# gopi-erabati/Object-Pose-Estimation

Measured on NVIDIA B200. Metric: frames_per_sec_fpfh_sacia_icp_640x480, higher is better.
Workload: dtype f32

## Files before the change

object-pose-estimation_b200/csrc/registration.cu:

```cuda
#include <cooperative_groups.h>

#include <algorithm>
#include <cmath>
#include <cstdlib>

#include <map>
#include <mutex>

#include <chrono>
#include "ope_host.cuh"
#include "ope_octet.cuh"

namespace cg = cooperative_groups;

namespace ope {

__global__ void transform_kernel(const float4* __restrict__ in, const float4* __restrict__ in_n, int n, Mat4 T,
                                 float4* __restrict__ out, float4* __restrict__ out_n) {
  int i = blockIdx.x * blockDim.x + threadIdx.x;
  if (i >= n) return;
  float4 p = __ldg(in + i);
  float4 o = p;
  xform_point(T, p.x, p.y, p.z, o.x, o.y, o.z);
  out[i] = o;
// ... 201 lines not shown
  float cert_gap;
  int dfs_max;
  int tgt_in_smem;
  int n_tgt;
  int split_min;
  int small_max;
  float4* def_q;
  int4* def_m;
  float4* def_res;
  int* def_count;
  int* def_head;
  double* partials;
  unsigned* barrier;
  ope_reg_result* result;
  long long* phase_cycles;
  Mat4 guess;
};

static constexpr int kIcpThreads = 512;
static constexpr int kIcpWarps = kIcpThreads / 32;
static constexpr int kIcpAcc = 17;
static constexpr int kIcpMaxBlocks = 1024;
static constexpr int kIcpSmemMaxTargets = 4096;
static constexpr int kIcpSplitMin = 6144;


struct IcpSmem {
  OctStack wstack[kIcpWarps];
  float2 knn_buf[kIcpWarps][kKnnBufCap + 32];
  LeafList leaves[kIcpWarps];
  int dir[kDirEntries];
  Nn1Smem<kIcpThreads> nn;
  double red[kIcpWarps][kIcpAcc];
  double totals[kIcpAcc];
  int prefix[2][kIcpMaxBlocks];
  int warp_cnt[2][kIcpWarps];
  int n_def[2];
  Mat4 T_inc;
  int stop;
};

__device__ __forceinline__ void grid_barrier(unsigned* counter, unsigned target) {
  __syncthreads();
  if (threadIdx.x == 0) {
    asm volatile("red.release.gpu.global.add.u32 [%0], 1;" ::"l"(counter) : "memory");
    unsigned v;
    do {
      asm volatile("ld.acquire.gpu.global.u32 %0, [%1];" : "=r"(v) : "l"(counter) : "memory");
    } while (v < target);
  }
  __syncthreads();
}

__device__ __forceinline__ double warp_reduce16(const double* v, int lane, int& slot) {
  double w8[8], w4[4], w2[2], w1;
  const bool b16 = lane & 16, b8 = lane & 8, b4 = lane & 4, b2 = lane & 2;
#pragma unroll
  for (int j = 0; j < 8; ++j) {
    const double keep = b16 ? v[j + 8] : v[j], give = b16 ? v[j] : v[j + 8];
    w8[j] = keep + __shfl_xor_sync(0xffffffffu, give, 16);
  }
#pragma unroll
  for (int j = 0; j < 4; ++j) {
    const double keep = b8 ? w8[j + 4] : w8[j], give = b8 ? w8[j] : w8[j + 4];
    w4[j] = keep + __shfl_xor_sync(0xffffffffu, give, 8);
  }
#pragma unroll
  for (int j = 0; j < 2; ++j) {
    const double keep = b4 ? w4[j + 2] : w4[j], give = b4 ? w4[j] : w4[j + 2];
    w2[j] = keep + __shfl_xor_sync(0xffffffffu, give, 4);
  }
  {
    const double keep = b2 ? w2[1] : w2[0], give = b2 ? w2[0] : w2[1];
    w1 = keep + __shfl_xor_sync(0xffffffffu, give, 2);
  }
  w1 += __shfl_xor_sync(0xffffffffu, w1, 1);
  slot = (b16 ? 8 : 0) + (b8 ? 4 : 0) + (b4 ? 2 : 0) + (b2 ? 1 : 0);
  return w1;
}

__device__ __forceinline__ double moment_term(int e, const float4 p, const float4 t, float d2, const double o[3]) {
  if (e == 0) return 1.0;
  if (e < 4) return e == 1 ? (double)p.x - o[0] : (e == 2 ? (double)p.y - o[1] : (double)p.z - o[2]);
  if (e < 7) return e == 4 ? (double)t.x - o[0] : (e == 5 ? (double)t.y - o[1] : (double)t.z - o[2]);
  if (e < 16) {
    const int c = (e - 7) / 3, r = (e - 7) % 3;
    const double sv = c == 0 ? (double)p.x - o[0] : (c == 1 ? (double)p.y - o[1] : (double)p.z - o[2]);
    const double tv = r == 0 ? (double)t.x - o[0] : (r == 1 ? (double)t.y - o[1] : (double)t.z - o[2]);
    return tv * sv;
  }
  return (double)d2;
}

__device__ __forceinline__ int icp_reject(const IcpDev& a, int s, int orig, const float4 p, int match) {
  const bool stale = a.variant == OPE_ICP_VARIANT_MODCORR;
  for (int r = 0; r < a.n_rej && match >= 0; ++r) {
    const float4 sn = stale ? __ldg(a.src0_nrm + orig) : a.cur_nrm[s];
    double score;
    if (a.rej_kind[r] == OPE_REJ_SURFACE_NORMAL) {
      const float4 tn = __ldg(a.tgt_nrm + match);
      score = (double)((sn.x * tn.x) + (sn.y * tn.y) + (sn.z * tn.z));
    } else {
      const float4 sp = stale ? __ldg(a.src0_pts + orig) : p;
      const double sl = (double)sqrtf(sp.x * sp.x + sp.y * sp.y + sp.z * sp.z);
      score = (double)((sn.x * (-sp.x / sl)) + (sn.y * (-sp.y / sl)) + (sn.z * (-sp.z / sl)));
    }
    if (!(score > a.rej_thr[r])) match = -1;
  }
  return match;
}

__device__ __forceinline__ int icp_gate(const IcpDev& a, int s, int orig, const float4 p, int nn, float d2) {
  int match = nn;
  if (match >= 0 && (double)d2 > a.max_corr_dist * a.max_corr_dist) match = -1;
  if (match >= 0) match = icp_reject(a, s, orig, p, match);
  return match;
}

__device__ __forceinline__ int icp_correspond_shooting(const IcpDev& a, OctStack* st, int s, int orig, const float4 p, bool use_seed,
                                                       float& d2_out, const float4* tg_smem = nullptr, float2* knn_buf = nullptr) {
  const unsigned full = 0xffffffffu;
  const int lane = threadIdx.x & 31;
  const bool ok = finite3(p.x, p.y, p.z);
  const bool stale = a.variant == OPE_ICP_VARIANT_MODCORR;
  const int k = a.k_search < a.grid.n ? a.k_search : a.grid.n;
  float bound = FLT_MAX;
  if (use_seed && ok) {
    int pj = -1;
    if (lane < k) pj = a.seed[(size_t)s * a.k_search + lane];
    float d = 0.0f;
    if (pj >= 0) { const float4 t = tg_smem ? tg_smem[pj] : __ldg(a.tgt_pts + pj); d = dist2(p.x, p.y, p.z, t.x, t.y, t.z); }
// ... 410 lines not shown
            const double cos_angle = 0.5 * (double)(T(0, 0) + T(1, 1) + T(2, 2) - 1);
            const double translation_sqr = (double)(T(0, 3) * T(0, 3) + T(1, 3) * T(1, 3) + T(2, 3) * T(2, 3));
            int hit = 0, hit_state = 0;
            if (cos_angle >= a.rot_thr && translation_sqr <= a.trans_thr) { hit = 1; hit_state = OPE_CONV_TRANSFORM; }
            else {
              cur_mse = sm->totals[16] / (double)n_corr;
              if (fabs(cur_mse - prev_mse) < a.abs_mse_thr) { hit = 1; hit_state = OPE_CONV_ABS_MSE; }
              else if (fabs(cur_mse - prev_mse) / prev_mse < a.rel_mse_thr) { hit = 1; hit_state = OPE_CONV_REL_MSE; }
              else prev_mse = cur_mse;
            }
            if (hit) {
              if (similar < a.max_similar) ++similar;
              else { similar = 0; state = hit_state; conv = 1; }
            }
          }
          converged = conv;
          if (a.force_all && iterations < a.max_iterations) conv = 0;
          if (conv) stop = 1;
        }
      }
      if (lane == 0) sm->stop = stop;
    }
    __syncthreads();
    if (prof) { const long long t1 = clock64(); t_phase[5] += t1 - t0; t0 = t1; }
    const int stop = sm->stop;
    if (stop != 2) {
      const Mat4 T = sm->T_inc;
      if (!shooting) { for (int s = lo + (int)threadIdx.x; s < hi; s += kIcpThreads) icp_move(a, T, s); }
      else { for (int s = wlo + lane; s < whi; s += 32) icp_move(a, T, s); __syncwarp(); }
    }
    if (prof) {
      const long long t1 = clock64(); t_phase[6] += t1 - t0;
      if (pass < 64) for (int k = 0; k < 7; ++k) { a.phase_cycles[16 + pass * 8 + k] = t_phase[k] - t_prev[k]; t_prev[k] = t_phase[k]; }
    }
    if (stop) break;
  }
  if (prof) {
    for (int i = 0; i < 7; ++i) a.phase_cycles[i] = t_phase[i];
    a.phase_cycles[7] = n_far;
  }
  if (blockIdx.x == 0 && threadIdx.x == 0) {
    ope_reg_result r;
    for (int i = 0; i < 16; ++i) r.T[i] = final_t.m[i];
    r.converged = converged; r.state = state; r.iterations = iterations; r.n_correspondences = n_corr;
    r.last_mse = cur_mse; r.best_error = 0.0; r.best_iteration = 0; r.reserved = 0;
    *a.result = r;
  }
}

static constexpr int kSlabSlots = 32;
static constexpr int kIcpSmallMaxBlocks = 32;

static constexpr int kIcpSmallThreads = 128;
template <int THREADS>
__device__ __forceinline__ void heap_sift(float2* column, int i, float2 v, const int n) {
  for (;;) {
    const int l = 2 * i + 1;
    if (l >= n) break;
    float2 cv = column[l * THREADS];
    int pick = l;
    if (l + 1 < n) {
      const float2 cr = column[(l + 1) * THREADS];
      if (nb_less(cv.x, __float_as_int(cv.y), cr.x, __float_as_int(cr.y))) { cv = cr; pick = l + 1; }
    }
    if (!nb_less(v.x, __float_as_int(v.y), cv.x, __float_as_int(cv.y))) break;
    column[i * THREADS] = cv;
    i = pick;
  }
  column[i * THREADS] = v;
}

template <int THREADS>
struct IcpSmallSmem {
  double red[THREADS / 32][kIcpAcc];
  double totals[kIcpAcc];
  float2 knn_buf[THREADS / 32][kKnnBufCap + 32];
  float4 wbox[THREADS / 32][2];
  Mat4 T_inc;
  int stop;
};

template <int THREADS>
__device__ __forceinline__ void icp_small_body(const IcpDev& a, const int bid, const int nblk) {
  constexpr int kIcpThreads = THREADS, kIcpWarps = THREADS / 32;
  extern __shared__ __align__(16) unsigned char smem_raw[];
  double morg[3];
  { const float4 t0 = a.n_tgt > 0 ? __ldg(a.tgt_pts) : make_float4(0, 0, 0, 0); moment_origin(t0.x, t0.y, t0.z, morg[0], morg[1], morg[2]); }
  IcpSmallSmem<THREADS>* sm = reinterpret_cast<IcpSmallSmem<THREADS>*>(smem_raw);
  float4* tg = reinterpret_cast<float4*>(smem_raw + ((sizeof(IcpSmallSmem<THREADS>) + 15) & ~(size_t)15));
  const int n_tgt8 = (a.n_tgt + 7) & ~7, n_groups = n_tgt8 >> 3;
  float4* blo = tg + n_tgt8;
  float4* bhi = blo + n_groups;
  float2* slab = reinterpret_cast<float2*>(bhi + n_groups);
  const unsigned full = 0xffffffffu;
  const int tid = threadIdx.x, lane = tid & 31, warp = tid >> 5;
  const int s = bid * kIcpThreads + tid;
  const bool in_range = s < a.n_work;
  const bool stale = a.variant == OPE_ICP_VARIANT_MODCORR;
  const int k = a.k_search < a.grid.n ? a.k_search : a.grid.n;
  auto col = [&](int slot) -> float2& { return slab[slot * kIcpThreads + tid]; };

  float4 p = make_float4(0, 0, 0, 0), nv = make_float4(0, 0, 0, 0);
  int orig = 0;
  if (in_range) {
    p = __ldg(a.src_sorted + s);
    orig = __float_as_int(p.w);
    if (a.src0_nrm) nv = __ldg(a.src0_nrm + orig);
    if (!mat4_is_identity(a.guess)) {
      float x, y, z;
      xform_point(a.guess, p.x, p.y, p.z, x, y, z);
      p.x = x; p.y = y; p.z = z;
      if (a.src0_nrm && finite3(nv.x, nv.y, nv.z)) { xform_normal(a.guess, nv.x, nv.y, nv.z, x, y, z); nv.x = x; nv.y = y; nv.z = z; }
    }
  }
  for (int j = tid; j < n_tgt8; j += kIcpThreads) tg[j] = j < a.n_tgt ? __ldg(a.tgt_pts + j) : make_float4(INFINITY, INFINITY, INFINITY, 0.0f);
  __syncthreads();
  for (int g = tid; g < n_groups; g += kIcpThreads) {
    float4 lo = make_float4(INFINITY, INFINITY, INFINITY, 0.0f), hi = make_float4(-INFINITY, -INFINITY, -INFINITY, 0.0f);
    for (int u = 0; u < 8; ++u) {
      const float4 t = tg[8 * g + u];
      if (!finite3(t.x, t.y, t.z)) continue;
      lo.x = fminf(lo.x, t.x); lo.y = fminf(lo.y, t.y); lo.z = fminf(lo.z, t.z);
      hi.x = fmaxf(hi.x, t.x); hi.y = fmaxf(hi.y, t.y); hi.z = fmaxf(hi.z, t.z);
    }
    blo[g] = lo; bhi[g] = hi;
  }
  __syncthreads();
  const bool ok = in_range && k > 0 && finite3(p.x, p.y, p.z);

  Mat4 final_t = a.guess;
  double prev_mse = DBL_MAX, cur_mse = DBL_MAX;
  int similar = 0, iterations = 0, state = OPE_CONV_NOT_CONVERGED, converged = 0, n_corr = 0;
  unsigned bar_target = 0;
  const bool prof = a.phase_cycles != nullptr && bid == 0 && tid == 0;
  long long t_phase[4] = {0, 0, 0, 0};

  auto coop_query = [&](int q, float bound) {
    const float qx = __shfl_sync(full, p.x, q), qy = __shfl_sync(full, p.y, q), qz = __shfl_sync(full, p.z, q);
    float ld; int li;
    const int cnt = warp_knn_smem_bounded(tg, a.n_tgt, a.grid.n, true, qx, qy, qz, a.k_search, bound, sm->knn_buf[warp], ld, li);
    float2* c = slab + (warp * 32 + q);
    if (lane < kSlabSlots) c[lane * kIcpThreads] = lane < cnt ? make_float2(ld, __int_as_float(li)) : make_float2(FLT_MAX, __int_as_float(-1));
    return cnt;
  };

  for (int pass = 0;; ++pass) {
    long long t0 = prof ? clock64() : 0;
    int c = 0;
    bool have = false;
    bool seeded = pass > 0;
    if (pass == 0) {
      const bool leader = (lane & 7) == 0;
      const unsigned lead = __ballot_sync(full, ok && leader);
      for (unsigned m = lead; m != 0u; m &= m - 1u) { const int q = __ffs(m) - 1; const int cnt = coop_query(q, FLT_MAX); if (lane == q) { c = cnt; have = true; } }
      __syncwarp();
      seeded = !leader && ((lead >> (lane & ~7)) & 1u);
    }
    float bound = FLT_MAX;
    if (ok && !have && seeded) {
      const float2* seed_col = slab + (pass == 0 ? (tid & ~7) : tid);
      float b = 0.0f;
      bool all = true;
#pragma unroll 4
      for (int j = 0; j < k; ++j) {
        const int idx = __float_as_int(seed_col[j * kIcpThreads].y);
        if (idx < 0) { all = false; continue; }
        const float4 t = tg[idx];
        b = fmaxf(b, dist2(p.x, p.y, p.z, t.x, t.y, t.z));
      }
      if (all) bound = b;
    }
    if (pass == 0) __syncwarp();
    const bool scan = ok && !have && bound < FLT_MAX;
    int n_ins = 0;
    bool heaped = false;
    float2 root = make_float2(0.0f, 0.0f);
    const long long ts0 = a.phase_cycles ? clock64() : 0;
    if (__any_sync(full, scan)) {
      auto insert_full = [&](float d2, int j) {
        ++n_ins;
        if (!heaped) {
          for (int i = kSlabSlots / 2 - 1; i >= 0; --i) heap_sift<THREADS>(slab + tid, i, col(i), kSlabSlots);
          heaped = true;
          root = col(0);
          bound = root.x;
        }
        if (nb_less(d2, j, root.x, __float_as_int(root.y))) {
          heap_sift<THREADS>(slab + tid, 0, make_float2(d2, __int_as_float(j)), kSlabSlots);
          root = col(0);
          bound = root.x;
        }
      };
      float wlx = scan ? p.x : INFINITY, wly = scan ? p.y : INFINITY, wlz = scan ? p.z : INFINITY;
      float whx = scan ? p.x : -INFINITY, why = scan ? p.y : -INFINITY, whz = scan ? p.z : -INFINITY;
      float wb = scan ? bound : 0.0f;
#pragma unroll
      for (int o = 16; o > 0; o >>= 1) {
        wlx = fminf(wlx, __shfl_xor_sync(full, wlx, o)); wly = fminf(wly, __shfl_xor_sync(full, wly, o)); wlz = fminf(wlz, __shfl_xor_sync(full, wlz, o));
        whx = fmaxf(whx, __shfl_xor_sync(full, whx, o)); why = fmaxf(why, __shfl_xor_sync(full, why, o)); whz = fmaxf(whz, __shfl_xor_sync(full, whz, o));
        wb = fmaxf(wb, __shfl_xor_sync(full, wb, o));
      }
      if (lane == 0) { sm->wbox[warp][0] = make_float4(wlx, wly, wlz, wb * 1.0002f + 1e-30f); sm->wbox[warp][1] = make_float4(whx, why, whz, 0.0f); }
      __syncwarp();
      for (int g0 = 0; g0 < n_groups; g0 += 32) {
        bool near = false;
        if (g0 + lane < n_groups) {
          const float4 lo = blo[g0 + lane], hi = bhi[g0 + lane], wl = sm->wbox[warp][0], wh = sm->wbox[warp][1];
          const float ex = fmaxf(fmaxf(lo.x - wh.x, wl.x - hi.x), 0.0f), ey = fmaxf(fmaxf(lo.y - wh.y, wl.y - hi.y), 0.0f),
                      ez = fmaxf(fmaxf(lo.z - wh.z, wl.z - hi.z), 0.0f);
          near = ex * ex + ey * ey + ez * ez <= wl.w;
        }
        for (unsigned cand = __ballot_sync(full, near); cand != 0u; cand &= cand - 1u) {
          const int g = g0 + __ffs(cand) - 1;
          const int j0 = 8 * g;
          bool mine = scan;
          if (mine) {
            const float4 lo = blo[g], hi = bhi[g];
            const float ex = fmaxf(fmaxf(lo.x - p.x, p.x - hi.x), 0.0f), ey = fmaxf(fmaxf(lo.y - p.y, p.y - hi.y), 0.0f),
                        ez = fmaxf(fmaxf(lo.z - p.z, p.z - hi.z), 0.0f);
            mine = ex * ex + ey * ey + ez * ez <= bound * 1.0001f + 1e-30f;
          }
          if (!mine) continue;
          float d2[8];
#pragma unroll
          for (int u = 0; u < 8; ++u) { const float4 t = tg[j0 + u]; d2[u] = dist2(p.x, p.y, p.z, t.x, t.y, t.z); }
          unsigned hit = 0u;
#pragma unroll
          for (int u = 0; u < 8; ++u) hit |= (d2[u] <= bound ? 1u : 0u) << u;
          if (hit == 0u) continue;
          if (c + __popc(hit) <= kSlabSlots) {
#pragma unroll
            for (int u = 0; u < 8; ++u)
              if ((hit >> u) & 1u) { col(c) = make_float2(d2[u], __int_as_float(j0 + u)); ++c; }
          } else {
#pragma unroll
            for (int u = 0; u < 8; ++u) {
              const bool h = (hit >> u) & 1u;
              const bool room = c < kSlabSlots;
              if (h & room) col(c) = make_float2(d2[u], __int_as_float(j0 + u));
              if (h & !room) insert_full(d2[u], j0 + u);
              c += (h & room) ? 1 : 0;
            }
          }
        }
      }
    }
    const bool unserved = ok && !have && (!scan || c < k);
    const unsigned redo = __ballot_sync(full, unserved);
    if (a.phase_cycles && pass < 64) {
      unsigned long long* pc = (unsigned long long*)(a.phase_cycles + 16 + pass * 8);
      const unsigned long long dt = (unsigned long long)(clock64() - ts0);
      if (lane == 0) { atomicAdd(pc + 0, dt); atomicMax(pc + 1, dt); atomicAdd(pc + 5, 1ull); }
      if (n_ins > 0) { atomicAdd(pc + 2, (unsigned long long)n_ins); atomicAdd(pc + 3, 1ull); }
      if (ok) atomicAdd(pc + 4, (unsigned long long)c);
    }
    if (a.phase_cycles && bid == 0 && lane == 0 && pass > 0) atomicAdd((unsigned long long*)&a.phase_cycles[4], (unsigned long long)__popc(redo));
    if (a.phase_cycles && bid == 0 && ok && pass > 0) atomicAdd((unsigned long long*)&a.phase_cycles[5], (unsigned long long)c);
    for (unsigned m = redo; m != 0u; m &= m - 1u) {
      const int q = __ffs(m) - 1;
      const float bq = __shfl_sync(full, scan ? bound : FLT_MAX, q);
      const int cnt = coop_query(q, bq);
      if (lane == q) c = cnt;
    }
    __syncwarp();
    if (prof) { const long long t1 = clock64(); t_phase[0] += t1 - t0; t0 = t1; }
    int match = -1;
    float d2m = 0.0f;
    if (ok && c > 0) {
      const float4 nr = stale ? __ldg(a.src0_nrm + orig) : nv;
      const double N0 = nr.x, N1 = nr.y, N2 = nr.z;
      double best = DBL_MAX;
      int best_idx = -1, first_idx = -1;
      float best_d2 = 0.0f, first_d2 = 0.0f;
      while (heaped && c > k) {
        --c;
        if (c > 0) heap_sift<THREADS>(slab + tid, 0, col(c), c);
      }
      while (c > k) {
        int worst = 0;
        float2 wv = col(0);
        for (int e = 1; e < c; ++e) { const float2 o = col(e); if (nb_less(wv.x, __float_as_int(wv.y), o.x, __float_as_int(o.y))) { wv = o; worst = e; } }
        --c;
        if (worst != c) col(worst) = col(c);
      }
      float best_key = 0.0f;
#pragma unroll 4
      for (int e = 0; e < c; ++e) {
        const float2 mine = col(e);
        const int mi = __float_as_int(mine.y);
        if (first_idx < 0 || nb_less(mine.x, mi, first_d2, first_idx)) { first_idx = mi; first_d2 = mine.x; }
        const float4 t = tg[mi];
        const float px = t.x - p.x, py = t.y - p.y, pz = t.z - p.z;
        const double V0 = px, V1 = py, V2 = pz;
        const double C0 = N1 * V2 - N2 * V1, C1 = N2 * V0 - N0 * V2, C2 = N0 * V1 - N1 * V0;
        const double dist = C0 * C0 + C1 * C1 + C2 * C2;
        if (dist < DBL_MAX && (dist < best || (dist == best && nb_less(mine.x, mi, best_key, best_idx)))) {
          best = dist; best_idx = mi; best_d2 = mine.x; best_key = mine.x;
        }
      }
      const int pick_idx = best_idx < 0 ? first_idx : best_idx;
      const float pick_d2 = best_idx < 0 ? first_d2 : best_d2;
      const double min_dist = best_idx < 0 ? DBL_MAX : best;
      if (!(min_dist > a.max_corr_dist)) { match = pick_idx; d2m = pick_d2; }
      for (int r = 0; r < a.n_rej && match >= 0; ++r) {
        const float4 sn = stale ? __ldg(a.src0_nrm + orig) : nv;
        double score;
        if (a.rej_kind[r] == OPE_REJ_SURFACE_NORMAL) {
          const float4 tn = __ldg(a.tgt_nrm + match);
          score = (double)((sn.x * tn.x) + (sn.y * tn.y) + (sn.z * tn.z));
        } else {
          const float4 sp = stale ? __ldg(a.src0_pts + orig) : p;
          const double sl = (double)sqrtf(sp.x * sp.x + sp.y * sp.y + sp.z * sp.z);
          score = (double)((sn.x * (-sp.x / sl)) + (sn.y * (-sp.y / sl)) + (sn.z * (-sp.z / sl)));
        }
        if (!(score > a.rej_thr[r])) match = -1;
      }
    }
    if (ok) for (int j = (c < k ? c : k); j < k; ++j) col(j) = make_float2(FLT_MAX, __int_as_float(-1));
    if (in_range) { a.corr_match[orig] = match; a.corr_d2[orig] = d2m; }
    if (prof) { const long long t1 = clock64(); t_phase[1] += t1 - t0; t0 = t1; }
    {
      double v[16];
#pragma unroll
      for (int e = 0; e < 16; ++e) v[e] = 0.0;
      double dsum = 0.0;
      if (match >= 0) {
        const float4 t = tg[match];
#pragma unroll
        for (int e = 0; e < 16; ++e) v[e] = moment_term(e, p, t, d2m, morg);
        dsum = (double)d2m;
      }
      int slot;
      const double wsum = warp_reduce16(v, lane, slot);
      dsum = warp_sum_d(dsum);
      if ((lane & 1) == 0) sm->red[warp][slot] = wsum;
      if (lane == 1) sm->red[warp][16] = dsum;
    }
    __syncthreads();
    double* my_partials = a.partials + ((size_t)(pass & 1) * nblk + bid) * kIcpAcc;
    if (tid < kIcpAcc) {
      double sum = 0.0;
#pragma unroll
      for (int wv = 0; wv < kIcpWarps; ++wv) sum += sm->red[wv][tid];
      my_partials[tid] = sum;
    }
    if (nblk > 1) { bar_target += nblk; grid_barrier(a.barrier, bar_target); } else __syncthreads();
    if (tid < kIcpAcc) {
      const double* base = a.partials + (size_t)(pass & 1) * nblk * kIcpAcc;
      double sum = 0.0;
      for (int b0 = 0; b0 < nblk; b0 += 8) {
        double v[8];
#pragma unroll
        for (int u = 0; u < 8; ++u) v[u] = b0 + u < nblk ? __ldcg(base + (size_t)(b0 + u) * kIcpAcc + tid) : 0.0;
#pragma unroll
        for (int u = 0; u < 8; ++u) sum += v[u];
      }
      sm->totals[tid] = sum;
    }
    __syncthreads();
    if (prof) { const long long t1 = clock64(); t_phase[2] += t1 - t0; t0 = t1; }
    if (tid == 0) {
      int stop = 0;
      n_corr = (int)sm->totals[0];
      if (n_corr < a.min_corr) {
        state = OPE_CONV_NO_CORRESPONDENCES; converged = 0; stop = 2;
        sm->T_inc = mat4_identity();
      } else {
        Mat4 T;
        umeyama_from_moments(sm->totals, T, morg[0], morg[1], morg[2]);
        sm->T_inc = T;
        final_t = mat4_mul(T, final_t);
        ++iterations;
        state = OPE_CONV_NOT_CONVERGED;
        int conv = 0;
        if (iterations >= a.max_iterations) {
          if (!a.fail_after_max) { state = OPE_CONV_ITERATIONS; conv = 1; }
          else { conv = 0; stop = 1; }
        } else {
          const double cos_angle = 0.5 * (double)(T(0, 0) + T(1, 1) + T(2, 2) - 1);
          const double translation_sqr = (double)(T(0, 3) * T(0, 3) + T(1, 3) * T(1, 3) + T(2, 3) * T(2, 3));
          int hit = 0, hit_state = 0;
          if (cos_angle >= a.rot_thr && translation_sqr <= a.trans_thr) { hit = 1; hit_state = OPE_CONV_TRANSFORM; }
          else {
            cur_mse = sm->totals[16] / (double)n_corr;
            if (fabs(cur_mse - prev_mse) < a.abs_mse_thr) { hit = 1; hit_state = OPE_CONV_ABS_MSE; }
            else if (fabs(cur_mse - prev_mse) / prev_mse < a.rel_mse_thr) { hit = 1; hit_state = OPE_CONV_REL_MSE; }
            else prev_mse = cur_mse;
          }
          if (hit) {
            if (similar < a.max_similar) ++similar;
            else { similar = 0; state = hit_state; conv = 1; }
          }
        }
        converged = conv;
        if (a.force_all && iterations < a.max_iterations) conv = 0;
        if (conv) stop = 1;
      }
      sm->stop = stop;
    }
    __syncthreads();
    const int stop = sm->stop;
    if (stop != 2 && in_range && finite3(p.x, p.y, p.z)) {
      const Mat4 T = sm->T_inc;
      float x, y, z;
      xform_point(T, p.x, p.y, p.z, x, y, z);
      p.x = x; p.y = y; p.z = z;
      if (a.src0_nrm && finite3(nv.x, nv.y, nv.z)) { xform_normal(T, nv.x, nv.y, nv.z, x, y, z); nv.x = x; nv.y = y; nv.z = z; }
    }
    if (prof) { const long long t1 = clock64(); t_phase[3] += t1 - t0; }
    if (stop) break;
  }
  if (prof) for (int i = 0; i < 4; ++i) a.phase_cycles[i] = t_phase[i];
  if (bid == 0 && tid == 0) {
    ope_reg_result r;
    for (int i = 0; i < 16; ++i) r.T[i] = final_t.m[i];
    r.converged = converged; r.state = state; r.iterations = iterations; r.n_correspondences = n_corr;
    r.last_mse = cur_mse; r.best_error = 0.0; r.best_iteration = 0; r.reserved = 0;
    *a.result = r;
  }
}

template <int THREADS>
__global__ void __launch_bounds__(THREADS, 512 / THREADS) icp_small_kernel(IcpDev a) {
  icp_small_body<THREADS>(a, (int)blockIdx.x, (int)gridDim.x);
}
template <int THREADS>
__global__ void __launch_bounds__(THREADS, 512 / THREADS) icp_small_batch_kernel(const IcpDev* __restrict__ descs, const int2* __restrict__ map,
                                                                                unsigned* ticket) {
  __shared__ int s_ticket;
  __shared__ IcpDev s_desc;
  if (threadIdx.x == 0) s_ticket = (int)atomicAdd(ticket, 1u);
  __syncthreads();
  const int2 fb = map[s_ticket];
  for (int w = threadIdx.x; w < (int)(sizeof(IcpDev) / 4); w += THREADS) reinterpret_cast<int*>(&s_desc)[w] = reinterpret_cast<const int*>(descs + fb.x)[w];
  __syncthreads();
  icp_small_body<THREADS>(s_desc, fb.y, (s_desc.n_work + THREADS - 1) / THREADS);
}

__global__ void __launch_bounds__(kIcpThreads, 1) correspond_once_kernel(IcpDev a) {
  extern __shared__ __align__(16) unsigned char smem_raw[];
  IcpSmem* sm = reinterpret_cast<IcpSmem*>(smem_raw);
  const int lane = threadIdx.x & 31, warp = threadIdx.x >> 5;
  if (a.estimator != OPE_EST_NORMAL_SHOOTING) {
    for (int base = blockIdx.x * kIcpThreads; base < a.n_src; base += gridDim.x * kIcpThreads) {
      const int i = base + (int)threadIdx.x;
      const bool in_range = i < a.n_src;
      float4 p = make_float4(0, 0, 0, 0);
      if (in_range) p = a.cur_pts[i];
      const bool ok = in_range && finite3(p.x, p.y, p.z);
      float d2 = 0.0f;
      const int nn = block_nn1<kIcpThreads>(a.grid, &sm->nn, ok, p.x, p.y, p.z, a.max_d2_f, -1, nullptr, d2);
      if (in_range) {
        const int m = ok ? icp_gate(a, i, i, p, nn, d2) : -1;
        a.corr_match[i] = m; a.corr_d2[i] = d2;
      }
    }
  } else {
    OctStack* st = &sm->wstack[warp];
    for (int i = blockIdx.x * kIcpWarps + warp; i < a.n_src; i += gridDim.x * kIcpWarps) {
      const float4 p = a.cur_pts[i];
      float d2 = 0.0f;
      const int m = icp_correspond_shooting(a, st, i, i, p, false, d2);
      if (lane == 0) { a.corr_match[i] = m; a.corr_d2[i] = d2; }
      __syncwarp();
    }
  }
}

__global__ void __launch_bounds__(kIcpThreads, 1) reciprocal_filter_kernel(GridView gsrc, const float4* __restrict__ tgt_pts, int* match,
                                                                           int n, float max_d2_f, double max_corr_dist) {
  extern __shared__ __align__(16) unsigned char smem_raw[];
  IcpSmem* sm = reinterpret_cast<IcpSmem*>(smem_raw);
  for (int base = blockIdx.x * kIcpThreads; base < n; base += gridDim.x * kIcpThreads) {
    const int i = base + (int)threadIdx.x;
    const int m = i < n ? match[i] : -1;
    float4 q = make_float4(0, 0, 0, 0);
    if (m >= 0) q = __ldg(tgt_pts + m);
    const bool ok = m >= 0 && finite3(q.x, q.y, q.z);
    float d2 = 0.0f;
    const int back = block_nn1<kIcpThreads>(gsrc, &sm->nn, ok, q.x, q.y, q.z, max_d2_f, -1, nullptr, d2);
// ... 544 lines not shown
}

static int icp_stepwise_device(ope_ctx* ctx, const ope_cloud* src, const ope_cloud* tgt, const ope_icp_params& prm, const Mat4& guess,
                               ope_reg_result* res, ope_correspondence* out_corr_host, ope_cloud** out_aligned,
                               ope_correspondence* fixed = nullptr, size_t n_fixed = 0);

int icp_device(ope_ctx* ctx, const ope_cloud* src, const ope_cloud* tgt, const ope_icp_params& prm, const Mat4& guess,
               ope_reg_result* res, ope_correspondence* out_corr_host, ope_cloud** out_aligned) {
  if (prm.transformation != OPE_TE_SVD || prm.use_reciprocal)
    return icp_stepwise_device(ctx, src, tgt, prm, guess, res, out_corr_host, out_aligned);
  IcpDev a;
  std::memset(&a, 0, sizeof(a));
  OPE_TRY(icp_fill(ctx, src, tgt, prm, &a, true));
  a.guess = guess;
  size_t smem_bytes = ((sizeof(IcpSmem) + 15) & ~(size_t)15) + (a.tgt_in_smem ? tgt->n * sizeof(float4) : 0);
  const size_t n = src->n;
  GridView gsrc;
  std::memset(&gsrc, 0, sizeof(gsrc));
  if (n > 0) OPE_TRY(cloud_any_grid(ctx, src, &gsrc));
  a.src_sorted = gsrc.pts;
  a.n_work = gsrc.n;
  const size_t nw = (size_t)a.n_work;
  ope_cloud* work = nullptr;
  OPE_TRY(cloud_alloc(ctx, std::max<size_t>(n, 1), src->normals != nullptr, &work));
  work->n = n;
  a.cur_pts = work->pts; a.cur_nrm = work->normals;
  Scratch<int> match(ctx), seed(ctx), dcount(ctx), dhead(ctx);
  Scratch<float> d2(ctx);
  Scratch<float4> defq(ctx), refs(ctx), defres(ctx);
  Scratch<int4> defm(ctx);
  Scratch<double> partials(ctx);
  Scratch<unsigned> bar(ctx);
  Scratch<ope_reg_result> dres(ctx);
  const bool shooting = prm.estimator == OPE_EST_NORMAL_SHOOTING;
  int rc = match.alloc(n);
  if (rc == OPE_OK) rc = d2.alloc(n);
  if (rc == OPE_OK) rc = seed.alloc(shooting ? nw * (size_t)prm.k_search : nw);
  if (rc == OPE_OK && !shooting) rc = defq.alloc(nw);
  if (rc == OPE_OK && !shooting) rc = defm.alloc(nw);
  if (rc == OPE_OK && !shooting) rc = refs.alloc(nw);
  if (rc == OPE_OK && !shooting) rc = defres.alloc(nw);
  if (rc == OPE_OK) rc = dres.alloc(1);
  if (rc == OPE_OK) rc = bar.alloc(1);
  if (rc == OPE_OK && cudaMemsetAsync(bar.p, 0, sizeof(unsigned), ctx->stream) != cudaSuccess) rc = fail(ctx, OPE_ERR_CUDA, "memset failed");
  if (rc == OPE_OK && n > 0 && cudaMemsetAsync(match.p, 0xff, n * sizeof(int), ctx->stream) != cudaSuccess) rc = fail(ctx, OPE_ERR_CUDA, "memset failed");
  if (rc == OPE_OK && n > 0 && cudaMemsetAsync(d2.p, 0, n * sizeof(float), ctx->stream) != cudaSuccess) rc = fail(ctx, OPE_ERR_CUDA, "memset failed");
  const char* small_env = std::getenv("OPE_ICP_SMALL");
  const bool want_small = small_env ? std::atoi(small_env) != 0 : ctx->icp_prefer_small;
  const bool small = want_small && a.tgt_in_smem && shooting && nw > 0 && nw <= (size_t)kIcpSmallMaxBlocks * kIcpSmallThreads &&
                     prm.k_search <= kSlabSlots;
  const void* kernel = small ? (const void*)icp_small_kernel<kIcpSmallThreads> : (const void*)icp_kernel;
  const int threads = small ? kIcpSmallThreads : kIcpThreads;
  if (small) {
    const size_t nt8 = (tgt->n + 7) & ~(size_t)7;
    smem_bytes = ((sizeof(IcpSmallSmem<kIcpSmallThreads>) + 15) & ~(size_t)15) + nt8 * sizeof(float4) + (nt8 / 8) * 2 * sizeof(float4) +
                 (size_t)kSlabSlots * kIcpSmallThreads * sizeof(float2);
    const char* pad = std::getenv("OPE_ICP_SMALL_MIN_SMEM_KB");
    const size_t min_bytes = (size_t)(pad ? std::atoi(pad) : 0) << 10;
    if (smem_bytes < min_bytes) smem_bytes = min_bytes;
  }
  if (rc == OPE_OK) rc = dyn_smem(ctx, kernel, smem_bytes);
  int per_sm = 0;
  if (rc == OPE_OK && cudaOccupancyMaxActiveBlocksPerMultiprocessor(&per_sm, kernel, threads, smem_bytes) != cudaSuccess)
    rc = fail(ctx, OPE_ERR_CUDA, "occupancy query failed");
  int blocks = 1;
  if (rc == OPE_OK && small) {
    if (per_sm < 1) rc = fail(ctx, OPE_ERR_CUDA, "icp_small_kernel cannot be resident");
    blocks = (int)((nw + kIcpSmallThreads - 1) / kIcpSmallThreads);
  } else if (rc == OPE_OK) {
    if (per_sm < 1) rc = fail(ctx, OPE_ERR_CUDA, "icp_kernel cannot be resident");
    int max_blocks = std::min(per_sm * ctx->sm_count, kIcpMaxBlocks);
    if (ctx->icp_max_blocks > 0) max_blocks = std::min(max_blocks, ctx->icp_max_blocks);
    const size_t want = shooting ? (nw + kIcpWarps - 1) / kIcpWarps : (nw + 127) / 128;
    blocks = (int)std::min<size_t>(std::max<size_t>(1, want), (size_t)max_blocks);
  }
  if (rc == OPE_OK) rc = partials.alloc((size_t)2 * blocks * kIcpAcc);
  if (rc == OPE_OK) rc = dcount.alloc((size_t)2 * blocks);
  if (rc == OPE_OK) rc = dhead.alloc(4);
  if (rc == OPE_OK && cudaMemsetAsync(dhead.p, 0, 4 * sizeof(int), ctx->stream) != cudaSuccess) rc = fail(ctx, OPE_ERR_CUDA, "memset failed");
  Scratch<long long> phases(ctx);
  const bool profile = std::getenv("OPE_PROFILE") != nullptr;
  const size_t n_prof = 16 + 64 * 8 + 64 + 64 * 4;
  if (rc == OPE_OK && profile) {
    rc = phases.alloc(n_prof); a.phase_cycles = phases.p;
    if (rc == OPE_OK) cudaMemsetAsync(phases.p, 0, n_prof * sizeof(long long), ctx->stream);
  }
  a.corr_match = match.p; a.corr_d2 = d2.p; a.seed = seed.p; a.def_q = defq.p; a.def_m = defm.p; a.def_count = dcount.p;
  a.ref = refs.p; a.def_head = dhead.p; a.def_res = defres.p;
  {
    const char* g = std::getenv("OPE_ICP_CERT_GAP");
    a.cert_gap = (g ? (float)std::atof(g) : 0.5f) * a.grid.h;
    const char* d = std::getenv("OPE_ICP_DFS_MAX");
    a.dfs_max = d ? std::atoi(d) : 0;
    const char* sp_ = std::getenv("OPE_ICP_SPLIT_MIN");
    a.split_min = sp_ ? std::atoi(sp_) : kIcpSplitMin;
    const char* sm_ = std::getenv("OPE_ICP_SMALL_MAX");
    a.small_max = sm_ ? std::atoi(sm_) : 0;
  }
  a.partials = partials.p; a.barrier = bar.p; a.result = dres.p;
  if (rc == OPE_OK) {
    void* args[] = {(void*)&a};
    cudaEventRecord(ctx->kev[0][0], ctx->stream);
    cudaError_t e = cudaLaunchCooperativeKernel(kernel, dim3(blocks), dim3(threads), args, smem_bytes, ctx->stream);
    cudaEventRecord(ctx->kev[0][1], ctx->stream);
    ctx->kev_valid[0] = true;
    if (e != cudaSuccess) rc = fail(ctx, OPE_ERR_CUDA, "cooperative launch of icp_kernel failed: %s", cudaGetErrorString(e));
    else rc = check_launch(ctx, "icp_kernel");
  }
  if (rc == OPE_OK) {
// ... 541 lines not shown
    max_nt = std::max(max_nt, (size_t)frames[i].n_tgt);
    total_src += (size_t)frames[i].n_src;
    total_blocks += ((size_t)frames[i].n_src + THREADS - 1) / THREADS;
  }
  Scratch<int> match(ctx);
  Scratch<float> d2(ctx);
  Scratch<double> partials(ctx);
  Scratch<unsigned> bars(ctx);
  Scratch<IcpDev> d_descs(ctx);
  Scratch<int2> d_map(ctx);
  OPE_TRY(match.alloc(total_src)); OPE_TRY(d2.alloc(total_src));
  OPE_TRY(partials.alloc(2 * total_blocks * kIcpAcc));
  OPE_TRY(bars.alloc((size_t)n_frames + 1));
  OPE_TRY(d_descs.alloc((size_t)n_frames)); OPE_TRY(d_map.alloc(total_blocks));
  OPE_CUDA_TRY(ctx, cudaMemsetAsync(bars.p, 0, ((size_t)n_frames + 1) * sizeof(unsigned), ctx->stream));
  size_t so = 0, bo = 0;
  map.reserve(total_blocks);
  for (int i = 0; i < n_frames; ++i) {
    IcpDev& a = descs[(size_t)i];
    std::memset(&a, 0, sizeof(a));
    const IcpBatchFrame& f = frames[i];
    a.grid.n = f.n_tgt;
    a.tgt_in_smem = 1; a.n_tgt = f.n_tgt;
    a.tgt_pts = f.tgt_pts; a.tgt_nrm = f.tgt_nrm;
    a.src0_pts = f.src_pts; a.src0_nrm = f.src_nrm; a.src_sorted = f.src_pts;
    a.n_src = f.n_src; a.n_work = f.n_src;
    a.max_iterations = prm.max_iterations; a.min_corr = prm.min_number_correspondences;
    a.estimator = prm.estimator; a.k_search = prm.k_search; a.n_rej = prm.n_rejectors;
    a.transformation = prm.transformation; a.variant = prm.variant; a.force_all = prm.force_all_iterations;
    for (int r = 0; r < OPE_MAX_REJECTORS; ++r) { a.rej_kind[r] = prm.rejector_kind[r]; a.rej_thr[r] = prm.rejector_threshold[r]; }
    a.max_corr_dist = prm.max_correspondence_distance;
    const double m2 = prm.max_correspondence_distance * prm.max_correspondence_distance;
    a.max_d2_f = (m2 >= (double)FLT_MAX || !(m2 == m2)) ? FLT_MAX : (float)m2;
    a.rot_thr = 1.0 - prm.transformation_epsilon; a.trans_thr = prm.transformation_epsilon;
    a.rel_mse_thr = prm.euclidean_fitness_epsilon; a.abs_mse_thr = prm.mse_threshold_absolute;
    a.max_similar = prm.max_iterations_similar_transforms; a.fail_after_max = prm.failure_after_max_iterations;
    a.guess = mat4_identity();
    const int nblk = (f.n_src + THREADS - 1) / THREADS;
    a.corr_match = match.p + so; a.corr_d2 = d2.p + so;
    a.partials = partials.p + 2 * bo * kIcpAcc;
    a.barrier = bars.p + i;
    a.result = d_results + i;
    for (int b = 0; b < nblk; ++b) map.push_back(make_int2(i, b));
    so += (size_t)f.n_src; bo += (size_t)nblk;
  }
  for (int r = 0; r < prm.n_rejectors; ++r)
    if (prm.rejector_kind[r] != OPE_REJ_SURFACE_NORMAL && prm.rejector_kind[r] != OPE_REJ_SELF_OCCLUDED_NORMAL)
      return fail(ctx, OPE_ERR_UNSUPPORTED, "unknown correspondence rejector kind %d", prm.rejector_kind[r]);
  OPE_CUDA_TRY(ctx, cudaMemcpyAsync(d_descs.p, descs.data(), descs.size() * sizeof(IcpDev), cudaMemcpyHostToDevice, ctx->stream));
  OPE_CUDA_TRY(ctx, cudaMemcpyAsync(d_map.p, map.data(), map.size() * sizeof(int2), cudaMemcpyHostToDevice, ctx->stream));
  const double t_prep = ms_since(t_enter);
  OPE_CUDA_TRY(ctx, ope::stream_sync(ctx));
  if (trace) fprintf(stderr, "[ope batch] icp launch: host preparation %.3f ms, then %.3f ms until the stream had drained\n", t_prep, ms_since(t_enter) - t_prep);
  const size_t nt8 = (max_nt + 7) & ~(size_t)7;
  const size_t smem_bytes = ((sizeof(IcpSmallSmem<THREADS>) + 15) & ~(size_t)15) + nt8 * sizeof(float4) + (nt8 / 8) * 2 * sizeof(float4) +
                            (size_t)kSlabSlots * THREADS * sizeof(float2);
  const void* kernel = (const void*)icp_small_batch_kernel<THREADS>;
  OPE_TRY(dyn_smem(ctx, kernel, smem_bytes));
  int per_sm = 0;
  OPE_CUDA_TRY(ctx, cudaOccupancyMaxActiveBlocksPerMultiprocessor(&per_sm, kernel, THREADS, smem_bytes));
  if ((size_t)per_sm * ctx->sm_count < (size_t)kIcpSmallMaxBlocks) return fail(ctx, OPE_ERR_CUDA, "icp_small_batch_kernel: one alignment's blocks cannot be co-resident");
  cudaEventRecord(ctx->kev[0][0], ctx->stream);
  icp_small_batch_kernel<THREADS><<<(unsigned)total_blocks, THREADS, smem_bytes, ctx->stream>>>(d_descs.p, d_map.p, bars.p + n_frames);
  cudaEventRecord(ctx->kev[0][1], ctx->stream);
  ctx->kev_valid[0] = true;
  return check_launch(ctx, "icp_small_batch_kernel");
}

int icp_small_batch_device(ope_ctx* ctx, const ope_icp_params& prm, const IcpBatchFrame* frames, int n_frames, ope_reg_result* d_results) {
  const char* e = std::getenv("OPE_ICP_BATCH_THREADS");
  const int t = e ? std::atoi(e) : 256;
  if (t == 128) return icp_small_batch_launch<128>(ctx, prm, frames, n_frames, d_results);
  return icp_small_batch_launch<256>(ctx, prm, frames, n_frames, d_results);
}

}

using namespace ope;

extern "C" {

void ope_icp_params_default(ope_icp_params* p) {
  std::memset(p, 0, sizeof(*p));
  p->max_iterations = 10;
  p->transformation_epsilon = 0.0;
  p->euclidean_fitness_epsilon = -DBL_MAX;
  p->max_correspondence_distance = std::sqrt(DBL_MAX);
  p->min_number_correspondences = 3;
  p->estimator = OPE_EST_NEAREST;
  p->k_search = 10;
  p->transformation = OPE_TE_SVD;
  p->variant = OPE_ICP_VARIANT_MOD;
  p->mse_threshold_absolute = 1e-12;
}
void ope_sacia_params_default(ope_sacia_params* p) {
  std::memset(p, 0, sizeof(*p));
  p->max_iterations = 10; p->nr_samples = 3; p->k_correspondences = 10; p->min_sample_distance = 0.0f;
  p->max_correspondence_distance = std::sqrt(DBL_MAX);
}
void ope_pose_params_default(ope_pose_params* p) {
  std::memset(p, 0, sizeof(*p));
  p->coarse_leaf = 0.01f; p->fine_leaf = 0.008f; p->normal_k = 30; p->fpfh_radius = 0.03f;
  ope_sacia_params_default(&p->sacia);
  p->sacia.max_iterations = 400; p->sacia.nr_samples = 5; p->sacia.k_correspondences = 5;
  p->sacia.min_sample_distance = 0.01f; p->sacia.max_correspondence_distance = 0.05;
  p->min_target_features = 10; p->min_target_points = 100;
  ope_icp_params_default(&p->icp);
  p->icp.max_iterations = 100; p->icp.transformation_epsilon = 1e-8; p->icp.euclidean_fitness_epsilon = 1e-8;
  p->icp.estimator = OPE_EST_NORMAL_SHOOTING; p->icp.k_search = 20;
  p->icp.n_rejectors = 2;
  p->icp.rejector_kind[0] = OPE_REJ_SURFACE_NORMAL; p->icp.rejector_threshold[0] = 0.7;
  p->icp.rejector_kind[1] = OPE_REJ_SELF_OCCLUDED_NORMAL; p->icp.rejector_threshold[1] = 0.6;
  p->icp.transformation = OPE_TE_SVD; p->icp.with_normals = 1;
  p->coarse_refit_threshold = 1e-4;
// ... 171 lines not shown
```

Before: 6670.

## Shrink ICP small-kernel register and shared footprint to raise occupancy

The kNN slab now stores 16-bit target indices instead of (distance, index) float2 pairs, and distances are recomputed from the shared-memory target cloud when needed. This cuts slab shared memory per block by a factor of four. Per-thread ICP state (final transform, MSE, counters, moment origin, profiling timers) moves into shared memory, and the 16-term moment vector is generated lazily inside the warp reduction instead of in a 16-double array. Together with raising the launch bound to 768/THREADS blocks per SM, this aims to lower register pressure and allow more resident blocks, at the cost of extra distance recomputation in the heap and selection loops.

```diff
diff --git a/object-pose-estimation_b200/csrc/registration.cu b/object-pose-estimation_b200/csrc/registration.cu
--- a/object-pose-estimation_b200/csrc/registration.cu
+++ b/object-pose-estimation_b200/csrc/registration.cu
@@ -277,12 +277,14 @@
   __syncthreads();
 }
 
-__device__ __forceinline__ double warp_reduce16(const double* v, int lane, int& slot) {
+template <class Term>
+__device__ __forceinline__ double warp_reduce16_terms(Term term, int lane, int& slot) {
   double w8[8], w4[4], w2[2], w1;
   const bool b16 = lane & 16, b8 = lane & 8, b4 = lane & 4, b2 = lane & 2;
 #pragma unroll
   for (int j = 0; j < 8; ++j) {
-    const double keep = b16 ? v[j + 8] : v[j], give = b16 ? v[j] : v[j + 8];
+    const double lo = term(j), hi = term(j + 8);
+    const double keep = b16 ? hi : lo, give = b16 ? lo : hi;
     w8[j] = keep + __shfl_xor_sync(0xffffffffu, give, 16);
   }
 #pragma unroll
@@ -302,6 +304,9 @@
   w1 += __shfl_xor_sync(0xffffffffu, w1, 1);
   slot = (b16 ? 8 : 0) + (b8 ? 4 : 0) + (b4 ? 2 : 0) + (b2 ? 1 : 0);
   return w1;
+}
+__device__ __forceinline__ double warp_reduce16(const double* v, int lane, int& slot) {
+  return warp_reduce16_terms([&](int e) { return v[e]; }, lane, slot);
 }
 
 __device__ __forceinline__ double moment_term(int e, const float4 p, const float4 t, float d2, const double o[3]) {
@@ -818,22 +823,28 @@
 static constexpr int kIcpSmallMaxBlocks = 32;
 
 static constexpr int kIcpSmallThreads = 128;
-template <int THREADS>
-__device__ __forceinline__ void heap_sift(float2* column, int i, float2 v, const int n) {
+typedef unsigned short SlabEntry;
+static constexpr SlabEntry kSlabEmpty = 0xffffu;
+static_assert(kIcpSmemMaxTargets <= kSlabEmpty, "target indices must fit a slab entry");
+
+template <int THREADS, class D2>
+__device__ __forceinline__ void heap_sift(SlabEntry* column, int i, float vd, int vi, const int n, D2 d2of) {
   for (;;) {
     const int l = 2 * i + 1;
     if (l >= n) break;
-    float2 cv = column[l * THREADS];
+    int ci = column[l * THREADS];
+    float cd = d2of(ci);
     int pick = l;
     if (l + 1 < n) {
-      const float2 cr = column[(l + 1) * THREADS];
-      if (nb_less(cv.x, __float_as_int(cv.y), cr.x, __float_as_int(cr.y))) { cv = cr; pick = l + 1; }
-    }
-    if (!nb_less(v.x, __float_as_int(v.y), cv.x, __float_as_int(cv.y))) break;
-    column[i * THREADS] = cv;
+      const int ri = column[(l + 1) * THREADS];
+      const float rd = d2of(ri);
+      if (nb_less(cd, ci, rd, ri)) { cd = rd; ci = ri; pick = l + 1; }
+    }
+    if (!nb_less(vd, vi, cd, ci)) break;
+    column[i * THREADS] = (SlabEntry)ci;
     i = pick;
   }
-  column[i * THREADS] = v;
+  column[i * THREADS] = (SlabEntry)vi;
 }
 
 template <int THREADS>
@@ -844,31 +855,47 @@
   float4 wbox[THREADS / 32][2];
   Mat4 T_inc;
   int stop;
+  Mat4 final_t;
+  double morg[3];
+  double prev_mse, cur_mse;
+  int similar, iterations, state, converged, n_corr;
+  long long t_phase[4], t_mark;
 };
+
+template <int THREADS>
+static size_t icp_small_smem_bytes(size_t n_tgt) {
+  const size_t nt8 = (n_tgt + 7) & ~(size_t)7;
+  return ((sizeof(IcpSmallSmem<THREADS>) + 15) & ~(size_t)15) + nt8 * sizeof(float4) + (nt8 / 8) * 2 * sizeof(float4) +
+         (size_t)kSlabSlots * THREADS * sizeof(SlabEntry);
+}
 
 template <int THREADS>
 __device__ __forceinline__ void icp_small_body(const IcpDev& a, const int bid, const int nblk) {
   constexpr int kIcpThreads = THREADS, kIcpWarps = THREADS / 32;
   extern __shared__ __align__(16) unsigned char smem_raw[];
-  double morg[3];
-  { const float4 t0 = a.n_tgt > 0 ? __ldg(a.tgt_pts) : make_float4(0, 0, 0, 0); moment_origin(t0.x, t0.y, t0.z, morg[0], morg[1], morg[2]); }
   IcpSmallSmem<THREADS>* sm = reinterpret_cast<IcpSmallSmem<THREADS>*>(smem_raw);
   float4* tg = reinterpret_cast<float4*>(smem_raw + ((sizeof(IcpSmallSmem<THREADS>) + 15) & ~(size_t)15));
   const int n_tgt8 = (a.n_tgt + 7) & ~7, n_groups = n_tgt8 >> 3;
   float4* blo = tg + n_tgt8;
   float4* bhi = blo + n_groups;
-  float2* slab = reinterpret_cast<float2*>(bhi + n_groups);
+  SlabEntry* slab = reinterpret_cast<SlabEntry*>(bhi + n_groups);
   const unsigned full = 0xffffffffu;
   const int tid = threadIdx.x, lane = tid & 31, warp = tid >> 5;
   const int s = bid * kIcpThreads + tid;
-  const bool in_range = s < a.n_work;
   const bool stale = a.variant == OPE_ICP_VARIANT_MODCORR;
   const int k = a.k_search < a.grid.n ? a.k_search : a.grid.n;
-  auto col = [&](int slot) -> float2& { return slab[slot * kIcpThreads + tid]; };
+  auto col = [&](int slot) -> SlabEntry& { return slab[slot * kIcpThreads + tid]; };
+  if (tid == 0) {
+    { const float4 t0 = a.n_tgt > 0 ? __ldg(a.tgt_pts) : make_float4(0, 0, 0, 0); moment_origin(t0.x, t0.y, t0.z, sm->morg[0], sm->morg[1], sm->morg[2]); }
+    sm->final_t = a.guess;
+    sm->prev_mse = DBL_MAX; sm->cur_mse = DBL_MAX;
+    sm->similar = 0; sm->iterations = 0; sm->state = OPE_CONV_NOT_CONVERGED; sm->converged = 0; sm->n_corr = 0;
+    for (int i = 0; i < 4; ++i) sm->t_phase[i] = 0;
+  }
 
   float4 p = make_float4(0, 0, 0, 0), nv = make_float4(0, 0, 0, 0);
-  int orig = 0;
-  if (in_range) {
+  int orig = -1;
+  if (s < a.n_work) {
     p = __ldg(a.src_sorted + s);
     orig = __float_as_int(p.w);
     if (a.src0_nrm) nv = __ldg(a.src0_nrm + orig);
@@ -892,26 +919,22 @@
     blo[g] = lo; bhi[g] = hi;
   }
   __syncthreads();
-  const bool ok = in_range && k > 0 && finite3(p.x, p.y, p.z);
-
-  Mat4 final_t = a.guess;
-  double prev_mse = DBL_MAX, cur_mse = DBL_MAX;
-  int similar = 0, iterations = 0, state = OPE_CONV_NOT_CONVERGED, converged = 0, n_corr = 0;
-  unsigned bar_target = 0;
+  const bool ok = orig >= 0 && k > 0 && finite3(p.x, p.y, p.z);
+  auto d2_to = [&](int j) { const float4 t = tg[j]; return dist2(p.x, p.y, p.z, t.x, t.y, t.z); };
+
   const bool prof = a.phase_cycles != nullptr && bid == 0 && tid == 0;
-  long long t_phase[4] = {0, 0, 0, 0};
 
   auto coop_query = [&](int q, float bound) {
     const float qx = __shfl_sync(full, p.x, q), qy = __shfl_sync(full, p.y, q), qz = __shfl_sync(full, p.z, q);
     float ld; int li;
     const int cnt = warp_knn_smem_bounded(tg, a.n_tgt, a.grid.n, true, qx, qy, qz, a.k_search, bound, sm->knn_buf[warp], ld, li);
-    float2* c = slab + (warp * 32 + q);
-    if (lane < kSlabSlots) c[lane * kIcpThreads] = lane < cnt ? make_float2(ld, __int_as_float(li)) : make_float2(FLT_MAX, __int_as_float(-1));
+    SlabEntry* c = slab + (warp * 32 + q);
+    if (lane < kSlabSlots) c[lane * kIcpThreads] = lane < cnt ? (SlabEntry)li : kSlabEmpty;
     return cnt;
   };
 
   for (int pass = 0;; ++pass) {
-    long long t0 = prof ? clock64() : 0;
+    if (prof) sm->t_mark = clock64();
     int c = 0;
     bool have = false;
     bool seeded = pass > 0;
@@ -924,13 +947,13 @@
     }
     float bound = FLT_MAX;
     if (ok && !have && seeded) {
-      const float2* seed_col = slab + (pass == 0 ? (tid & ~7) : tid);
+      const SlabEntry* seed_col = slab + (pass == 0 ? (tid & ~7) : tid);
       float b = 0.0f;
       bool all = true;
 #pragma unroll 4
       for (int j = 0; j < k; ++j) {
-        const int idx = __float_as_int(seed_col[j * kIcpThreads].y);
-        if (idx < 0) { all = false; continue; }
+        const int idx = seed_col[j * kIcpThreads];
+        if (idx == kSlabEmpty) { all = false; continue; }
         const float4 t = tg[idx];
         b = fmaxf(b, dist2(p.x, p.y, p.z, t.x, t.y, t.z));
       }
@@ -940,21 +963,24 @@
     const bool scan = ok && !have && bound < FLT_MAX;
     int n_ins = 0;
     bool heaped = false;
-    float2 root = make_float2(0.0f, 0.0f);
+    float root_d2 = 0.0f;
+    int root_i = 0;
     const long long ts0 = a.phase_cycles ? clock64() : 0;
     if (__any_sync(full, scan)) {
       auto insert_full = [&](float d2, int j) {
         ++n_ins;
         if (!heaped) {
-          for (int i = kSlabSlots / 2 - 1; i >= 0; --i) heap_sift<THREADS>(slab + tid, i, col(i), kSlabSlots);
+          for (int i = kSlabSlots / 2 - 1; i >= 0; --i) { const int vi = col(i); heap_sift<THREADS>(slab + tid, i, d2_to(vi), vi, kSlabSlots, d2_to); }
           heaped = true;
-          root = col(0);
-          bound = root.x;
+          root_i = col(0);
+          root_d2 = d2_to(root_i);
+          bound = root_d2;
         }
-        if (nb_less(d2, j, root.x, __float_as_int(root.y))) {
-          heap_sift<THREADS>(slab + tid, 0, make_float2(d2, __int_as_float(j)), kSlabSlots);
-          root = col(0);
-          bound = root.x;
+        if (nb_less(d2, j, root_d2, root_i)) {
+          heap_sift<THREADS>(slab + tid, 0, d2, j, kSlabSlots, d2_to);
+          root_i = col(0);
+          root_d2 = d2_to(root_i);
+          bound = root_d2;
         }
       };
       float wlx = scan ? p.x : INFINITY, wly = scan ? p.y : INFINITY, wlz = scan ? p.z : INFINITY;
@@ -997,13 +1023,13 @@
           if (c + __popc(hit) <= kSlabSlots) {
 #pragma unroll
             for (int u = 0; u < 8; ++u)
-              if ((hit >> u) & 1u) { col(c) = make_float2(d2[u], __int_as_float(j0 + u)); ++c; }
+              if ((hit >> u) & 1u) { col(c) = (SlabEntry)(j0 + u); ++c; }
           } else {
 #pragma unroll
             for (int u = 0; u < 8; ++u) {
               const bool h = (hit >> u) & 1u;
               const bool room = c < kSlabSlots;
-              if (h & room) col(c) = make_float2(d2[u], __int_as_float(j0 + u));
+              if (h & room) col(c) = (SlabEntry)(j0 + u);
               if (h & !room) insert_full(d2[u], j0 + u);
               c += (h & room) ? 1 : 0;
             }
@@ -1029,7 +1055,7 @@
       if (lane == q) c = cnt;
     }
     __syncwarp();
-    if (prof) { const long long t1 = clock64(); t_phase[0] += t1 - t0; t0 = t1; }
+    if (prof) { const long long t1 = clock64(); sm->t_phase[0] += t1 - sm->t_mark; sm->t_mark = t1; }
     int match = -1;
     float d2m = 0.0f;
     if (ok && c > 0) {
@@ -1040,28 +1066,28 @@
       float best_d2 = 0.0f, first_d2 = 0.0f;
       while (heaped && c > k) {
         --c;
-        if (c > 0) heap_sift<THREADS>(slab + tid, 0, col(c), c);
+        if (c > 0) { const int vi = col(c); heap_sift<THREADS>(slab + tid, 0, d2_to(vi), vi, c, d2_to); }
       }
       while (c > k) {
-        int worst = 0;
-        float2 wv = col(0);
-        for (int e = 1; e < c; ++e) { const float2 o = col(e); if (nb_less(wv.x, __float_as_int(wv.y), o.x, __float_as_int(o.y))) { wv = o; worst = e; } }
+        int worst = 0, wi = col(0);
+        float wd = d2_to(wi);
+        for (int e = 1; e < c; ++e) { const int oi = col(e); const float od = d2_to(oi); if (nb_less(wd, wi, od, oi)) { wd = od; wi = oi; worst = e; } }
         --c;
         if (worst != c) col(worst) = col(c);
       }
       float best_key = 0.0f;
 #pragma unroll 4
       for (int e = 0; e < c; ++e) {
-        const float2 mine = col(e);
-        const int mi = __float_as_int(mine.y);
-        if (first_idx < 0 || nb_less(mine.x, mi, first_d2, first_idx)) { first_idx = mi; first_d2 = mine.x; }
+        const int mi = col(e);
         const float4 t = tg[mi];
+        const float md = dist2(p.x, p.y, p.z, t.x, t.y, t.z);
+        if (first_idx < 0 || nb_less(md, mi, first_d2, first_idx)) { first_idx = mi; first_d2 = md; }
         const float px = t.x - p.x, py = t.y - p.y, pz = t.z - p.z;
         const double V0 = px, V1 = py, V2 = pz;
         const double C0 = N1 * V2 - N2 * V1, C1 = N2 * V0 - N0 * V2, C2 = N0 * V1 - N1 * V0;
         const double dist = C0 * C0 + C1 * C1 + C2 * C2;
-        if (dist < DBL_MAX && (dist < best || (dist == best && nb_less(mine.x, mi, best_key, best_idx)))) {
-          best = dist; best_idx = mi; best_d2 = mine.x; best_key = mine.x;
+        if (dist < DBL_MAX && (dist < best || (dist == best && nb_less(md, mi, best_key, best_idx)))) {
+          best = dist; best_idx = mi; best_d2 = md; best_key = md;
         }
       }
       const int pick_idx = best_idx < 0 ? first_idx : best_idx;
@@ -1082,23 +1108,15 @@
         if (!(score > a.rej_thr[r])) match = -1;
       }
     }
-    if (ok) for (int j = (c < k ? c : k); j < k; ++j) col(j) = make_float2(FLT_MAX, __int_as_float(-1));
-    if (in_range) { a.corr_match[orig] = match; a.corr_d2[orig] = d2m; }
-    if (prof) { const long long t1 = clock64(); t_phase[1] += t1 - t0; t0 = t1; }
+    if (ok) for (int j = (c < k ? c : k); j < k; ++j) col(j) = kSlabEmpty;
+    if (orig >= 0) { a.corr_match[orig] = match; a.corr_d2[orig] = d2m; }
+    if (prof) { const long long t1 = clock64(); sm->t_phase[1] += t1 - sm->t_mark; sm->t_mark = t1; }
     {
-      double v[16];
-#pragma unroll
-      for (int e = 0; e < 16; ++e) v[e] = 0.0;
-      double dsum = 0.0;
-      if (match >= 0) {
-        const float4 t = tg[match];
-#pragma unroll
-        for (int e = 0; e < 16; ++e) v[e] = moment_term(e, p, t, d2m, morg);
-        dsum = (double)d2m;
-      }
+      const bool has = match >= 0;
+      const float4 t = has ? tg[match] : make_float4(0, 0, 0, 0);
       int slot;
-      const double wsum = warp_reduce16(v, lane, slot);
-      dsum = warp_sum_d(dsum);
+      const double wsum = warp_reduce16_terms([&](int e) { return has ? moment_term(e, p, t, d2m, sm->morg) : 0.0; }, lane, slot);
+      const double dsum = warp_sum_d(has ? (double)d2m : 0.0);
       if ((lane & 1) == 0) sm->red[warp][slot] = wsum;
       if (lane == 1) sm->red[warp][16] = dsum;
     }
@@ -1110,7 +1128,7 @@
       for (int wv = 0; wv < kIcpWarps; ++wv) sum += sm->red[wv][tid];
       my_partials[tid] = sum;
     }
-    if (nblk > 1) { bar_target += nblk; grid_barrier(a.barrier, bar_target); } else __syncthreads();
+    if (nblk > 1) grid_barrier(a.barrier, (unsigned)(pass + 1) * (unsigned)nblk); else __syncthreads();
     if (tid < kIcpAcc) {
       const double* base = a.partials + (size_t)(pass & 1) * nblk * kIcpAcc;
       double sum = 0.0;
@@ -1124,8 +1142,11 @@
       sm->totals[tid] = sum;
     }
     __syncthreads();
-    if (prof) { const long long t1 = clock64(); t_phase[2] += t1 - t0; t0 = t1; }
+    if (prof) { const long long t1 = clock64(); sm->t_phase[2] += t1 - sm->t_mark; sm->t_mark = t1; }
     if (tid == 0) {
+      Mat4& final_t = sm->final_t;
+      double &prev_mse = sm->prev_mse, &cur_mse = sm->cur_mse;
+      int &similar = sm->similar, &iterations = sm->iterations, &state = sm->state, &converged = sm->converged, &n_corr = sm->n_corr;
       int stop = 0;
       n_corr = (int)sm->totals[0];
       if (n_corr < a.min_corr) {
@@ -1133,7 +1154,7 @@
         sm->T_inc = mat4_identity();
       } else {
         Mat4 T;
-        umeyama_from_moments(sm->totals, T, morg[0], morg[1], morg[2]);
+        umeyama_from_moments(sm->totals, T, sm->morg[0], sm->morg[1], sm->morg[2]);
         sm->T_inc = T;
         final_t = mat4_mul(T, final_t);
         ++iterations;
@@ -1166,22 +1187,22 @@
     }
     __syncthreads();
     const int stop = sm->stop;
-    if (stop != 2 && in_range && finite3(p.x, p.y, p.z)) {
+    if (stop != 2 && orig >= 0 && finite3(p.x, p.y, p.z)) {
       const Mat4 T = sm->T_inc;
       float x, y, z;
       xform_point(T, p.x, p.y, p.z, x, y, z);
       p.x = x; p.y = y; p.z = z;
       if (a.src0_nrm && finite3(nv.x, nv.y, nv.z)) { xform_normal(T, nv.x, nv.y, nv.z, x, y, z); nv.x = x; nv.y = y; nv.z = z; }
     }
-    if (prof) { const long long t1 = clock64(); t_phase[3] += t1 - t0; }
+    if (prof) { const long long t1 = clock64(); sm->t_phase[3] += t1 - sm->t_mark; sm->t_mark = t1; }
     if (stop) break;
   }
-  if (prof) for (int i = 0; i < 4; ++i) a.phase_cycles[i] = t_phase[i];
   if (bid == 0 && tid == 0) {
+    if (a.phase_cycles) for (int i = 0; i < 4; ++i) a.phase_cycles[i] = sm->t_phase[i];
     ope_reg_result r;
-    for (int i = 0; i < 16; ++i) r.T[i] = final_t.m[i];
-    r.converged = converged; r.state = state; r.iterations = iterations; r.n_correspondences = n_corr;
-    r.last_mse = cur_mse; r.best_error = 0.0; r.best_iteration = 0; r.reserved = 0;
+    for (int i = 0; i < 16; ++i) r.T[i] = sm->final_t.m[i];
+    r.converged = sm->converged; r.state = sm->state; r.iterations = sm->iterations; r.n_correspondences = sm->n_corr;
+    r.last_mse = sm->cur_mse; r.best_error = 0.0; r.best_iteration = 0; r.reserved = 0;
     *a.result = r;
   }
 }
@@ -1191,7 +1212,7 @@
   icp_small_body<THREADS>(a, (int)blockIdx.x, (int)gridDim.x);
 }
 template <int THREADS>
-__global__ void __launch_bounds__(THREADS, 512 / THREADS) icp_small_batch_kernel(const IcpDev* __restrict__ descs, const int2* __restrict__ map,
+__global__ void __launch_bounds__(THREADS, 768 / THREADS) icp_small_batch_kernel(const IcpDev* __restrict__ descs, const int2* __restrict__ map,
                                                                                 unsigned* ticket) {
   __shared__ int s_ticket;
   __shared__ IcpDev s_desc;
@@ -1842,9 +1863,7 @@
   const void* kernel = small ? (const void*)icp_small_kernel<kIcpSmallThreads> : (const void*)icp_kernel;
   const int threads = small ? kIcpSmallThreads : kIcpThreads;
   if (small) {
-    const size_t nt8 = (tgt->n + 7) & ~(size_t)7;
-    smem_bytes = ((sizeof(IcpSmallSmem<kIcpSmallThreads>) + 15) & ~(size_t)15) + nt8 * sizeof(float4) + (nt8 / 8) * 2 * sizeof(float4) +
-                 (size_t)kSlabSlots * kIcpSmallThreads * sizeof(float2);
+    smem_bytes = icp_small_smem_bytes<kIcpSmallThreads>(tgt->n);
     const char* pad = std::getenv("OPE_ICP_SMALL_MIN_SMEM_KB");
     const size_t min_bytes = (size_t)(pad ? std::atoi(pad) : 0) << 10;
     if (smem_bytes < min_bytes) smem_bytes = min_bytes;
@@ -2492,14 +2511,14 @@
   const double t_prep = ms_since(t_enter);
   OPE_CUDA_TRY(ctx, ope::stream_sync(ctx));
   if (trace) fprintf(stderr, "[ope batch] icp launch: host preparation %.3f ms, then %.3f ms until the stream had drained\n", t_prep, ms_since(t_enter) - t_prep);
-  const size_t nt8 = (max_nt + 7) & ~(size_t)7;
-  const size_t smem_bytes = ((sizeof(IcpSmallSmem<THREADS>) + 15) & ~(size_t)15) + nt8 * sizeof(float4) + (nt8 / 8) * 2 * sizeof(float4) +
-                            (size_t)kSlabSlots * THREADS * sizeof(float2);
+  const size_t smem_bytes = icp_small_smem_bytes<THREADS>(max_nt);
   const void* kernel = (const void*)icp_small_batch_kernel<THREADS>;
   OPE_TRY(dyn_smem(ctx, kernel, smem_bytes));
   int per_sm = 0;
   OPE_CUDA_TRY(ctx, cudaOccupancyMaxActiveBlocksPerMultiprocessor(&per_sm, kernel, THREADS, smem_bytes));
   if ((size_t)per_sm * ctx->sm_count < (size_t)kIcpSmallMaxBlocks) return fail(ctx, OPE_ERR_CUDA, "icp_small_batch_kernel: one alignment's blocks cannot be co-resident");
+  if (trace) fprintf(stderr, "[ope batch] icp launch: %d alignments, %zu blocks of %d threads, largest target %zu points, %zu B shared memory per block, %d blocks per SM\n",
+                     n_frames, total_blocks, THREADS, max_nt, smem_bytes, per_sm);
   cudaEventRecord(ctx->kev[0][0], ctx->stream);
   icp_small_batch_kernel<THREADS><<<(unsigned)total_blocks, THREADS, smem_bytes, ctx->stream>>>(d_descs.p, d_map.p, bars.p + n_frames);
   cudaEventRecord(ctx->kev[0][1], ctx->stream);
```

Result: faster. 6741 (median of 6 runs) (+1.1%).
